# JuanTarrio/rebvo

Hardware: AMD Instinct MI355X
Metric: frames/sec (DoG+extract+track+depth) 752x480 EuRoC (higher is better)
Workload: dtype f32 scale-space / f64 tracker+EKF

## Files before the change

### rebvo_amd/csrc/api.hip

```cpp

#include <math.h>
#include <stdio.h>
#include <stdlib.h>
#include <string.h>

#include <algorithm>
#include <mutex>

#include "ctx.h"
#include "stage_a_dev.h"

namespace edgehip {

static thread_local std::string g_err;

int wait_pinned_ring(edgehip_ctx *c) {
    const int r = c->frames_seen % 8;
    if (c->ring_valid[r]) EH_CHECK(hipEventSynchronize(c->ev_ring[r]));
    return 0;
}

static int wait_idx_row(edgehip_ctx *c, int slot, const int32_t *pi) {
    if (c->slot_src[slot].idx_row != pi) return 0;
    if (c->a_api_valid[slot]) EH_CHECK(hipEventSynchronize(c->ev_a[slot]));
// ... 424 lines not shown
    EH_TRY(dmalloc(c, &c->band_off, B * (nstrips + 1), al->dev, 0));
    {
        char *bs;
        EH_TRY(dmalloc(c, &bs, B * nstrips * c->band_cap * 20, al->dev));
        c->band_stage = bs;
    }
    EH_TRY(dmalloc(c, &c->histo, B * 256, al->dev, 0));
    c->nblk_tvr = (int)((CAP + kTvrBlock - 1) / kTvrBlock);
    EH_TRY(dmalloc(c, &c->P0, B * 3 * CAP, al->dev, 0));
    EH_TRY(dmalloc(c, &c->resid, (size_t)kResidBufs * B * CAP, al->dev, 0));
    EH_TRY(dmalloc(c, &c->resid_carry, (size_t)kResidBufs * B * c->nblk_tvr, al->dev, 0));
    EH_TRY(dmalloc(c, &c->partials, 2 * B * c->nblk_tvr * kNumSums, al->dev, 0));
    EH_TRY(dmalloc(c, &c->block_last, 2 * B * c->nblk_tvr, al->dev, 0));
    EH_TRY(dmalloc(c, &c->bin_cnt, B * 256, al->dev, 0));
    {
        const size_t ntiles = (size_t)((p.w + 63) / 64) * ((p.h + 63) / 64);
        EH_TRY(dmalloc(c, &c->bins, B * ntiles * CAP, al->dev));
    }
    c->field_radius = p.search_range;
    c->field_mode = EH_EXP_ENV("EDGEHIP_FIELD_MODE", 0);
    c->no_grec = getenv("EDGEHIP_NO_GREC") && atoi(getenv("EDGEHIP_NO_GREC")) != 0;
    c->level_mode = getenv("EDGEHIP_LEVEL_MODE") ? atoi(getenv("EDGEHIP_LEVEL_MODE")) : 0;
    c->fwd_mode = EH_EXP_ENV("EDGEHIP_FWD_MODE", 0);
    c->fused_min_batch = fused_min_env;
    c->fused_undist = EH_EXP_ENV("EDGEHIP_FUSED_UNDIST", 0) != 0;
    c->tvr_rw2 = EH_EXP_ENV("EDGEHIP_TVR_RW2", 0);
    c->dual_init = getenv("EDGEHIP_DUAL_INIT") ? atoi(getenv("EDGEHIP_DUAL_INIT")) : 1;
    c->persist_lm_max = EH_EXP_ENV("EDGEHIP_PERSIST_LM", 0);
    EH_TRY(dmalloc(c, &c->sync_cnt, B, al->dev, 0));
    EH_TRY(dmalloc(c, &c->fwd_key, B * CAP, al->dev, 0));
    EH_TRY(dmalloc(c, &c->fwd_win, B * CAP, al->dev, 0xFF));
    EH_TRY(dmalloc(c, &c->rs_tmp, B * 2 * CAP, al->dev, 0));
    c->fuse_match = !(getenv("EDGEHIP_FUSE_MATCH") && atoi(getenv("EDGEHIP_FUSE_MATCH")) == 0);
    if (c->fuse_match) {
        EH_TRY(dmalloc(c, &c->rot_pm, S * B * CAP, al->dev, 0)); EH_TRY(dmalloc(c, &c->rot_mm, S * B * CAP, al->dev, 0));
        EH_TRY(dmalloc(c, &c->rot_rho, S * B * CAP, al->dev, 0)); EH_TRY(dmalloc(c, &c->rot_srho, S * B * CAP, al->dev, 0));
    }
    EH_TRY(dmalloc(c, &c->rot_buf, B * 9, al->dev, 0));
    EH_TRY(dmalloc(c, &c->nav_dev, B, al->dev, 0));
    EH_TRY(dmalloc(c, &c->idx_dev, B, al->dev, 0));
    c->slot_src.assign(S, edgehip_ctx::SlotSrc());
    c->stereo_cnt = nullptr;
    if (p.stereo_available) EH_TRY(dmalloc(c, &c->stereo_cnt, B, al->dev, 0));
    c->nav_log = nullptr;
    c->nav_log_len = 0;

    {
        const size_t al256 = 256;
        auto up = [&](size_t x) { return (x + al256 - 1) / al256 * al256; };
        const bool stereo = p.stereo_available != 0;
        const size_t per = up(CAP * 4) * 8  +
                           up(CAP * 8) * 6  + up(CAP * 8) * 7  + up(CAP * 32) + up(CAP * 16)  +
                           (stereo ? up(CAP * 4) + 2 * up(CAP * 8) : 0);
        char *arena;
        EH_TRY(dmalloc(c, &arena, per * S * B, al->dev, 0));
        c->kl_arena = arena;
        c->kl.resize(S * B);
        for (size_t sb = 0; sb < S * B; sb++) {
            char *q = arena + sb * per;
            KlSoA &k = c->kl[sb];
            auto take = [&](size_t bytes) { char *r = q; q += up(bytes); return r; };
            k.p_inx = (int32_t *)take(CAP * 4);
            k.m_m = (float2 *)take(CAP * 8); k.u_m = (float2 *)take(CAP * 8); k.c_p = (float2 *)take(CAP * 8);
            k.p_m = (float2 *)take(CAP * 8); k.p_m_0 = (float2 *)take(CAP * 8); k.m_m0 = (float2 *)take(CAP * 8);
            k.n_m = (float *)take(CAP * 4);
            k.rho = (double *)take(CAP * 8); k.s_rho = (double *)take(CAP * 8); k.rho_nr = (double *)take(CAP * 8);
// ... 1029 lines not shown
```

### rebvo_amd/csrc/ctx.h

```cpp
#pragma once
#include <hip/hip_runtime.h>
#include <stdint.h>
#include <string.h>
#include <string>
#include <map>
#include <vector>
#include <mutex>
#include <atomic>

#include "edgehip.h"
#include "export_ring.h"

namespace edgehip {

constexpr int kMaxBoxes = 3;
constexpr int kBandRows = 12;
constexpr int kDetWaves = 16;
constexpr int kDivLutMax = 256;
constexpr int kTvrThreads = 256;
constexpr int kTvrPasses = 1;
constexpr int kTvrBlock = kTvrThreads * kTvrPasses;
constexpr int kNumSums = 28;
constexpr int kRefRing = 8;
constexpr int kResidBufs = 3;
// ... 358 lines not shown
    struct SlotSrc { const uint8_t *base = nullptr; std::vector<int32_t> host_idx; bool grey8 = false;
                     const int32_t *idx_row = nullptr; int idx_ring = 0; };
    uint8_t *grey8 = nullptr;
    uint8_t *pinned_grey8 = nullptr;
    std::vector<SlotSrc> slot_src;
    struct SlotCam { float ppx, ppy; double zfm; };
    std::vector<SlotCam> slot_cam;
    int field_radius;
    int field_mode;
    int level_mode;
    int fused_min_batch;
    double pinv_host[3 * 49];
    int32_t *bin_cnt;
    int32_t *bins;
    int nblk_tvr;
    bool fused_undist;
    int tvr_rw2;
    bool tracker_f32 = false;
    int dual_init;
    int persist_lm_max;
    unsigned *sync_cnt;
    unsigned long long *fwd_key;
    int32_t *fwd_win;
    int fwd_mode = 0;
    bool fuse_match = true;
    float2 *rot_pm = nullptr, *rot_mm = nullptr;
    double *rot_rho = nullptr, *rot_srho = nullptr;
    bool rot_pending[4] = {false, false, false, false};
    bool fwd_fill[4] = {false, false, false, false};
    bool fwd_cleared = false;
    bool fwd_keys_posted = false;
    bool fwd_key_in_tvr = false;
    double *rs_tmp;
    double *rot_buf;
    const double *t_src = nullptr;
    edgehip_keyline *aos_dev = nullptr;
    edgehip_keyline *aos_host = nullptr;
    int32_t *aos_req_dev = nullptr, *aos_req_host = nullptr;
    int aos_requests = 0;
    edgehip::ExportRing kl_ring;
    edgehip::ExportRing ros_ring;
    edgehip_nav *nav_dev;
    edgehip_nav *nav_log;
    edgehip_nav_imu *nav_imu_log = nullptr;
    int nav_log_len;
    int32_t *stereo_log = nullptr;
    hipStream_t stream_log = nullptr;
    hipEvent_t ev_log = nullptr;
    hipEvent_t ev_log_ring[8] = {};
    std::mutex log_mu;
    std::atomic<long long> frames_logged{0};
    long long log_first = 0, log_last = -1;
    int32_t *idx_dev;
    int32_t *stereo_cnt;
    uint8_t *pinned_rgb;
    size_t pinned_rgb_bytes;
    edgehip::SeqDev *pinned_seq;
    edgehip::SeqA *pinned_seqa;
    double *pinned_out;
    double *pinned_t;
    int32_t *pinned_idx;
    edgehip_nav *pinned_nav;
    edgehip::Profiler *prof;
    bool imu_enabled = false, imu_pending = false;
    bool imu_pinned_ok = false;
    edgehip_imu_params imu_params;
// ... 84 lines not shown
void drop_frame_graphs(edgehip_ctx *c);
int order_a_after_bc(edgehip_ctx *c);
int order_bc_after_a(edgehip_ctx *c);
int sync_all(edgehip_ctx *c);
int undistort_frame_enqueue(edgehip_ctx *c, int seq, int slot, uint8_t *out_dev);
__device__ inline void frame_begin(SeqDev *sq, double t, double fps) {
    edgehip_seq_state &p = sq->pub;
    double dt = t - p.t_prev;
    if (dt < 0.001) dt = 1 / fps;
    p.dt = dt;
    sq->t_cur = t;
    for (int i = 0; i < 9; i++) {
        const double d = (i == 0 || i == 4 || i == 8) ? 1.0 : 0.0;
        p.P_V[i] = d * 1e50; p.P_W[i] = d * 1e50; p.R[i] = d;
    }
    p.klm_fwd = 0; p.klm_num = 0; p.kf_matchs = 0;
    p.estimation_ok = 1;
    sq->skip_match = 0;
    sq->skip_map = 0;
    p.minimizer_evals = 0;
}

int quantile_enqueue(edgehip_ctx *c, int slot, double smin, double smax, double pct, int nbins, bool frame_begins = false, int retune_slot = -1);
int build_field_enqueue(edgehip_ctx *c, int slot, int radius, float min_mod, bool clear_fwd = false);
int tvr_prepare_enqueue(edgehip_ctx *c, int slot_old, unsigned begin_ops = 0);
int minimizer_enqueue(edgehip_ctx *c, int slot_new, int slot_old, int fc_index);
int minimizer_v_enqueue(edgehip_ctx *c, int slot_new, int slot_old, int fc_index, int iter_max, double match_thresh,
                         uint32_t match_num_thresh, double reweight_distance);
int forward_match_enqueue(edgehip_ctx *c, int slot_old, int slot_new, bool keys_posted = false, bool frame_tail = false);
int forward_rotate_enqueue(edgehip_ctx *c, int slot_old, int slot_new);
int rotate_enqueue(edgehip_ctx *c, int slot, const double *R_host, bool R_in_buf = false);
int rot_materialize_enqueue(edgehip_ctx *c, int slot);
int rec_refresh_enqueue(edgehip_ctx *c, int slot);
int directed_enqueue(edgehip_ctx *c, int slot_new, int slot_old, bool fused = false);
int regekf_enqueue(edgehip_ctx *c, int slot, int do_reg, int do_ekf, bool frame_glue = false);
int rescale_enqueue(edgehip_ctx *c, int slot, bool frame_ends = false);
int pose_enqueue(edgehip_ctx *c, int slot_new, const double *t_host);
int imu_begin_enqueue(edgehip_ctx *c);
int imu_reset_enqueue(edgehip_ctx *c);
int imu_pose_reset_enqueue(edgehip_ctx *c, int seq);
int imu_pre_enqueue(edgehip_ctx *c, int slot_old);
int imu_mid_enqueue(edgehip_ctx *c);
int imu_post_enqueue(edgehip_ctx *c, int slot_new, int have_pair);
void depth_fill_free(edgehip_ctx *c);
int depth_fill_geometry(edgehip_ctx *c, int32_t *gw, int32_t *gh, int32_t *bw, int32_t *bh);
bool depth_fill_grids(edgehip_ctx *c, const double **rho, const double **s_rho);
void depth_surface_free(edgehip_ctx *c);
void net_free(edgehip_ctx *c);
bool net_store(edgehip_ctx *c, const uint8_t **records, const edgehip_net_header **headers, int *kl_size);
void surface_views_free(edgehip_ctx *c);
void ros_free(edgehip_ctx *c);
void kf_track_free(edgehip_ctx *c);
int kf_track_reset_enqueue(edgehip_ctx *c);
int kf_frame_begin_enqueue(edgehip_ctx *c, int slot_old);
int kf_frame_track_enqueue(edgehip_ctx *c, int slot_new);
int kf_frame_end_enqueue(edgehip_ctx *c, int slot_new);

inline int slot_read_done(edgehip_ctx *c, int slot) {
    if (c->stream_a == c->stream) return 0;
    EH_CHECK(hipEventRecord(c->ev_use[slot], c->stream));
    c->use_valid[slot] = true;
    return 0;
}

struct KProfStage {
    double *dev = nullptr, *host = nullptr;
    hipEvent_t ev = nullptr;
    bool busy = false;
// ... 25 lines not shown
```

### rebvo_amd/csrc/stage_c.hip

```cpp

#include <math.h>
#include <string.h>

#include <vector>

#include "ctx.h"
#include "wave_reduce.h"

namespace edgehip {

constexpr double kRhoMax = 20.0, kRhoMin = 1e-3, kRhoInit = 1.0;

__global__ __launch_bounds__(256) void k_fwd_key(const KlSoA *kl_old, const int32_t *__restrict__ kn_old,
                                                 const int32_t *__restrict__ kn_new, unsigned long long *__restrict__ key,
                                                 int cap) {
    const int seq = blockIdx.z, i = blockIdx.x * 256 + threadIdx.x;
    if (i >= kn_old[seq]) return;
    const int f = kl_old[seq].m_id_f[i];
    if (f < 0 || f >= kn_new[seq]) return;
    atomicMax(&key[(size_t)seq * cap + f], ord_bits(kl_old[seq].rho[i]));
}
__device__ inline void so3_exp_c(const double w[3], double R[9]);
__device__ inline void rot_from_state(SeqDev *sq, double *__restrict__ Rbuf_seq);
__device__ inline void glue_after_tracking(SeqDev *sq);
// ... 275 lines not shown
        else { r2[0] = (M[2] + M[6]) / 2; r2[1] = (M[7] + M[5]) / 2; r2[2] = d2; }
        if (r2[0] * r[0] + r2[1] * r[1] + r2[2] * r[2] < 0) { r2[0] = -r2[0]; r2[1] = -r2[1]; r2[2] = -r2[2]; }
        const double nn = sqrt(r2[0] * r2[0] + r2[1] * r2[1] + r2[2] * r2[2]);
        for (int i = 0; i < 3; i++) r[i] = angle * (r2[i] / nn);
    }
}

__device__ inline void rot_from_state(SeqDev *sq, double *__restrict__ Rbuf_seq) {
    double R0[9];
    so3_exp_c(sq->pub.W, R0);
    for (int i = 0; i < 9; i++) Rbuf_seq[i] = R0[i];
    for (int i = 0; i < 3; i++)
        for (int j = 0; j < 3; j++) sq->pub.R[i * 3 + j] = R0[j * 3 + i];
}
__global__ void k_rot_from_state(SeqDev *seqs, double *__restrict__ Rbuf, int nseq) {
    const int seq = blockIdx.x * blockDim.x + threadIdx.x;
    if (seq >= nseq) return;
    rot_from_state(seqs + seq, Rbuf + (size_t)seq * 9);
}

struct DirArgs {
    const KlSoA *kl_new, *kl_old;
    const int32_t *kn_new;
    const int32_t *mask_old;
    SeqDev *seq;
    int w, h;
    size_t n;
    double zfm, min_thr_mod, cang_min_edge, max_radius, loc_unc;
    float ppx, ppy;
    int stereo_mode;
    const int32_t *win;
    RotOut rot;
    int cap;
};

#ifndef EDGEHIP_NT_ROT
#define EDGEHIP_NT_ROT 1
#endif
#ifndef EDGEHIP_NT_EKF
#define EDGEHIP_NT_EKF 1
#endif
#ifndef EDGEHIP_NT_DIRECTED
#define EDGEHIP_NT_DIRECTED 1
#endif
template <bool FUSED, bool FILL>
__device__ __forceinline__ void directed_body(const DirArgs &a) {
    const int seq = blockIdx.z, ik = blockIdx.x * (int)blockDim.x + threadIdx.x;
    SeqDev *sq = a.seq + seq;
    const bool searching = !sq->skip_match;
    if (!FUSED && !searching) return;
    __shared__ double s_v[3], s_rv[9], s_br[9];
    if (threadIdx.x == 0 && searching) {
        const double *BR = sq->pub.R, *V = sq->pub.V, *P = sq->pub.P_V;
        for (int i = 0; i < 9; i++) s_br[i] = BR[i];
        for (int i = 0; i < 3; i++) {
            double d = 0;
            for (int j = 0; j < 3; j++) d += BR[i * 3 + j] * V[j];
            s_v[i] = d;
        }
        double T[9];
        for (int i = 0; i < 3; i++)
            for (int j = 0; j < 3; j++) {
                double d = 0;
                for (int k = 0; k < 3; k++) d += BR[i * 3 + k] * P[k * 3 + j];
                T[i * 3 + j] = d;
            }
        for (int i = 0; i < 3; i++)
            for (int j = 0; j < 3; j++) {
                double d = 0;
                for (int k = 0; k < 3; k++) d += T[i * 3 + k] * BR[j * 3 + k];
                s_rv[i * 3 + j] = d;
            }
    }
    __syncthreads();
    int matched = 0, kfm = 0, fwd = 0;
    if (ik < a.kn_new[seq]) {
        const KlSoA &kn = a.kl_new[seq], &ko = a.kl_old[seq];
        const int32_t *mask = a.mask_old + (size_t)seq * a.n;
        const size_t ro = (size_t)seq * a.cap;
// ... 104 lines not shown
                    const double t = tv[c][dir];
                    jm[c][dir] = -1;
                    if (t0i + c >= t_end) continue;
                    if (dir ? t > dq_max : t < dq_min) continue;
                    const float fx = (float)(t_x * t + (double)pi0x), fy = (float)(t_y * t + (double)pi0y);
                    const int xi = round_half_away_i(fx), yi = round_half_away_i(fy);
                    if (xi >= a.w || yi >= a.h || xi < 0 || yi < 0) continue;
                    jm[c][dir] = mask[__umul24((unsigned)yi, (unsigned)a.w) + (unsigned)xi];
                }
            }
#pragma unroll
            for (int c = 0; c < DM_CH; c++) {
#pragma unroll
                for (int dir = 0; dir < 2; dir++) {
                    const int j = jm[c][dir];
                    if (j < 0 || found >= 0) continue;
                    const double t = tv[c][dir];
                    const float2 omm = FUSED ? ldg(a.rot.m_m, ro + j) : ldg(ko.m_m, j);
                    const double norm_m0 = (double)ldg(ko.n_m, j);
                    const double cang = div_mid((double)(omm.x * kmm.x + omm.y * kmm.y), norm_m0 * norm_m);
                    if (cang < a.cang_min_edge || fabs(norm_m0 / norm_m - 1) > a.min_thr_mod) continue;
                    const double s_rho = FUSED ? ldg(a.rot.s_rho, ro + j) : ldg(ko.s_rho, j), rho = FUSED ? ldg(a.rot.rho, ro + j) : ldg(ko.rho, j);
                    const double v_rho_dr = (a.loc_unc * a.loc_unc + s_rho * s_rho * norm_t * norm_t + sigma2_t * rho * rho);
                    const double dd = t - norm_t * rho;
                    if (dd * dd > v_rho_dr) continue;
                    found = j;
                }
            }
        }
        }
        }
        if (FUSED) {
            const int src = found >= 0 ? found : iw;
            if (src >= 0 || FILL) {
                double rho = kRhoInit, s_rho = kRhoMax, rho_nr = kRhoInit, s_rho_nr = kRhoMax;
                int32_t m_num = -1, m_id_kf = -1;
                float2 pm, mm = make_float2(0.f, 0.f);
                float nm = 0.f;
                if (src < 0) {
                    pm = ldg(kn.p_m, ik);
                } else {
                    const bool turned = found >= 0;
                    rho = turned ? ldg(a.rot.rho, ro + src) : ldg(ko.rho, src);
                    s_rho = turned ? ldg(a.rot.s_rho, ro + src) : ldg(ko.s_rho, src);
                    pm = turned ? ldg(a.rot.p_m, ro + src) : ldg(ko.p_m, src);
                    mm = turned ? ldg(a.rot.m_m, ro + src) : ldg(ko.m_m, src);
                    rho_nr = ldg(ko.rho_nr, src); s_rho_nr = ldg(ko.s_rho_nr, src);
                    m_num = ldg(ko.m_num, src); m_id_kf = ldg(ko.m_id_kf, src);
                    nm = ldg(ko.n_m, src);
                }
#if EDGEHIP_NT_DIRECTED
                stg_stream(kn.rho, ik, rho);
                stg_stream(kn.s_rho, ik, s_rho);
                stg_stream(kn.rho_nr, ik, rho_nr);
                stg_stream(kn.s_rho_nr, ik, s_rho_nr);
                stg_stream(kn.m_num, ik, m_num + 1);
                stg_stream(kn.m_id, ik, src);
                stg_stream(kn.p_m_0, ik, pm);
                stg_stream(kn.m_m0, ik, mm);
                stg_stream(kn.n_m0, ik, (double)nm);
                stg_stream(kn.m_id_kf, ik, m_id_kf);
#else
                stg(kn.rho, ik, rho);
                stg(kn.s_rho, ik, s_rho);
                stg(kn.rho_nr, ik, rho_nr);
                stg(kn.s_rho_nr, ik, s_rho_nr);
                stg(kn.m_num, ik, m_num + 1);
                stg(kn.m_id, ik, src);
                stg(kn.p_m_0, ik, pm);
                stg(kn.m_m0, ik, mm);
                stg(kn.n_m0, ik, (double)nm);
                stg(kn.m_id_kf, ik, m_id_kf);
#endif
                matched = found >= 0;
                kfm = matched && m_id_kf >= 0;
            }
        } else if (found >= 0) {
            const int j = found;
            const double c_rho = a.stereo_mode ? ldg(ko.rho0, j) : ldg(ko.rho, j), c_srho = a.stereo_mode ? ldg(ko.s_rho0, j) : ldg(ko.s_rho, j);
            double c_rho_nr = 0, c_srho_nr = 0;
            if (!a.stereo_mode) { c_rho_nr = ldg(ko.rho_nr, j); c_srho_nr = ldg(ko.s_rho_nr, j); }
            const int32_t c_mnum = ldg(ko.m_num, j), mk = ldg(ko.m_id_kf, j);
            const float2 c_pm = ldg(ko.p_m, j), c_mm = ldg(ko.m_m, j);
            const float c_nm = ldg(ko.n_m, j);
            stg(kn.rho, ik, c_rho);
            stg(kn.s_rho, ik, c_srho);
            if (!a.stereo_mode) {
                stg(kn.rho_nr, ik, c_rho_nr);
                stg(kn.s_rho_nr, ik, c_srho_nr);
            }
            stg(kn.m_id, ik, j);
            stg(kn.m_num, ik, c_mnum + 1);
            stg(kn.p_m_0, ik, c_pm);
            stg(kn.m_m0, ik, c_mm);
            stg(kn.n_m0, ik, (double)c_nm);
            stg(kn.m_id_kf, ik, mk);
            matched = 1;
            kfm = mk >= 0;
        }
    }
    const int c1 = __popcll(__ballot(matched)), c2 = __popcll(__ballot(kfm)), c3 = FUSED ? __popcll(__ballot(fwd)) : 0;
    if ((threadIdx.x & 63) == 0) {
        if (c1) atomicAdd(&sq->pub.klm_num, c1);
        if (c2) atomicAdd(&sq->pub.kf_matchs, c2);
        if (c3) atomicAdd(&sq->pub.klm_fwd, c3);
    }
}
__global__ __launch_bounds__(256) void k_directed(DirArgs a) { directed_body<false, false>(a); }
template <bool FILL>
__global__ __launch_bounds__(256) __attribute__((amdgpu_waves_per_eu(7, 8))) void k_directed_fused(DirArgs a) { directed_body<true, FILL>(a); }


__device__ inline void glue_after_matching(SeqDev *sq);
__global__ __launch_bounds__(256) void k_regularize(const KlSoA *kls, const int32_t *__restrict__ kns, double *__restrict__ rs,
                                                    SeqDev *seqs, int cap, double thresh, int enabled, int match_threshold) {
    const int seq = blockIdx.z, i = blockIdx.x * 256 + threadIdx.x;
    SeqDev *sq = seqs + seq;
    bool skip = sq->skip_map != 0;
    if (match_threshold >= 0 && !sq->skip_match && sq->pub.klm_num < match_threshold) {
        if (i == 0) glue_after_matching(sq);
        skip = true;
    }
    if (skip) return;
    if (i >= kns[seq]) return;
    const KlSoA &K = kls[seq];
    double r = ldg(K.rho, i), s = ldg(K.s_rho, i);
    const int ni = ldg(K.n_id, i), pi = ldg(K.p_id, i);
    if (enabled && ni >= 0 && pi >= 0) {
        const double nrho = ldg(K.rho, ni), prho = ldg(K.rho, pi), nsr = ldg(K.s_rho, ni), psr = ldg(K.s_rho, pi);
        const double d = nrho - prho;
        if (!(d * d > nsr * nsr + psr * psr)) {
            const float2 nm = ldg(K.m_m, ni), pm = ldg(K.m_m, pi);
            double alpha = (double)((nm.x * pm.x + nm.y * pm.y) / (ldg(K.n_m, ni) * ldg(K.n_m, pi)));
            if (!(alpha - thresh < 0)) {
                alpha = (alpha - thresh) / (1 - thresh);
                alpha /= fabs(nrho - prho) / (nsr + psr) + 1;
                const double wr = 1 / (s * s), wrn = alpha / (nsr * nsr), wrp = alpha / (psr * psr);
                const double r2 = (r * wr + nrho * wrn + prho * wrp) / (wr + wrn + wrp);
                const double s2 = (s * wr + nsr * wrn + psr * wrp) / (wr + wrn + wrp);
                r = r2;
                s = s2;
            }
        }
    }
    rs[(size_t)seq * 2 * cap + i] = r;
    rs[(size_t)seq * 2 * cap + cap + i] = s;
}

__global__ __launch_bounds__(256) void k_ekf(const KlSoA *kls, const int32_t *__restrict__ kns, const double *__restrict__ rs,
                                             const SeqDev *seqs, int cap, double zf, double q_abs, double loc_unc, int do_ekf) {
    const int seq = blockIdx.z, i = blockIdx.x * 256 + threadIdx.x;
    const SeqDev *sq = seqs + seq;
    if (sq->skip_map) return;
    if (i >= kns[seq]) return;
    const KlSoA &K = kls[seq];
    double rho = rs[(size_t)seq * 2 * cap + i], s_rho = rs[(size_t)seq * 2 * cap + cap + i];
    if (do_ekf && ldg(K.m_id, i) >= 0) {
        const double v0 = sq->pub.V[0], v1 = sq->pub.V[1], v2 = sq->pub.V[2];
        const double s_rho0 = s_rho;
        const float2 q = ldg(K.p_m, i), q0 = ldg(K.p_m_0, i), mm0 = ldg(K.m_m0, i);
        const double qx = q.x, qy = q.y, q0x = q0.x, q0y = q0.y;
        double v_rho = s_rho * s_rho;
        const double nm0 = ldg(K.n_m0, i);
        const double u_x = (double)mm0.x / nm0, u_y = (double)mm0.y / nm0;
        const double Y = u_x * (qx - q0x) + u_y * (qy - q0y);
        const double H = u_x * (v0 * zf - v2 * q0x) + u_y * (v1 * zf - v2 * q0y);
        const double rho_p = 1 / (1.0 / rho + v2);
        const double rho0 = rho_p;
        double F = 1 / (1 + rho * v2);
        F = F * F;
        const double p_p = F * v_rho * F + q_abs * q_abs;
        const double e = Y - H * rho_p;
        const double S = H * p_p * H + loc_unc * loc_unc;
        const double Kg = p_p * H * (1 / S);
        rho = rho_p + (Kg * e);
        v_rho = (1 - Kg * H) * p_p;
        s_rho = sqrt(v_rho);
        if (rho < kRhoMin) {
            s_rho += kRhoMin - rho;
            rho = kRhoMin;
        } else if (rho > kRhoMax) {
            rho = kRhoMax;
        } else if (isnan(rho) || isnan(s_rho) || isinf(rho) || isinf(s_rho)) {
            rho = kRhoInit;
            s_rho = kRhoMax;
        } else if (s_rho < 0) {
            rho = kRhoInit;
            s_rho = kRhoMax;
        }
#if EDGEHIP_NT_EKF
        stg_stream(K.rho0, i, rho0);
        stg_stream(K.s_rho0, i, s_rho0);
    }
    stg_stream(K.rho, i, rho);
    stg_stream(K.s_rho, i, s_rho);
#else
        stg(K.rho0, i, rho0);
        stg(K.s_rho0, i, s_rho0);
    }
    stg(K.rho, i, rho);
    stg(K.s_rho, i, s_rho);
#endif
}

__device__ __forceinline__ double recip_f64(double x) {
    double y = __builtin_amdgcn_rcp(x);
    y = __builtin_fma(__builtin_fma(-x, y, 1.0), y, y);
    y = __builtin_fma(__builtin_fma(-x, y, 1.0), y, y);
    return y;
}

struct FrameEndArgs {
    edgehip_nav *nav;
    const int32_t *kn_new;
    const double *tresh_new;
    const float *retuned_new;
    edgehip_nav *nav_log;
    int nav_log_len, nseq, have_pair;
};
__device__ inline void frame_end(SeqDev *sq, const int seq, const FrameEndArgs &fe);

template <int NT, int PER, int LJ>
__global__ __launch_bounds__(NT) void k_rescale(const KlSoA *kls, const int32_t *__restrict__ kns, SeqDev *seqs,
                                                double s_rho_min, unsigned match_num_min, int re_escale, FrameEndArgs fe) {
    constexpr int VT = 1024 / NT;
    extern __shared__ double s_tail[];
    const int seq = blockIdx.x, tid = threadIdx.x;
    SeqDev *sq = seqs + seq;
    const int kn = kns[seq];
    bool run = !sq->skip_map;
    if (run && kn <= 0) { if (tid == 0) sq->pub.Kp = 1; run = false; }
    if (run) {
    const KlSoA &K = kls[seq];
    __shared__ double s_a[16], s_b[16];
    __shared__ double s_kp;
    double r2[VT][PER], r02[VT][PER], s2[VT][PER], s02[VT][PER];
// ... 520 lines not shown
                              uy * zf1 * (a.t[1] * den - a.t[2] * (qh1[1] + a.t[1] * srho)) / (den * den);
            double I_rho = (df / a.loc_unc_model) * (df / a.loc_unc_model);
            if (srho != srho || df != df) { srho = 1; I_rho = 1e-10; }
            double ss = 1 / sqrt(I_rho);
            if (srho < 0) { ss = 1e3; srho = 1.0; match = -1; }
            k.stereo_rho[i] = srho;
            k.stereo_s_rho[i] = ss;
        }
        k.stereo_m_id[i] = match;
        matched = match >= 0;
    }
    const int c1 = __popcll(__ballot(matched));
    if ((threadIdx.x & 63) == 0 && c1) atomicAdd(&a.nmatch[seq], c1);
}

__global__ __launch_bounds__(256) void k_fuse_stereo(const KlSoA *kls, const int32_t *__restrict__ kns, SeqDev *seqs) {
    const int seq = blockIdx.z, i = blockIdx.x * 256 + threadIdx.x;
    if (seqs) {
        if (seqs[seq].skip_map) return;
        if (i == 0) seqs[seq].pub.Kp = 1;
    }
    if (i >= kns[seq]) return;
    const KlSoA &k = kls[seq];
    const double r0 = k.rho[i], s0 = k.s_rho[i];
    k.rho0[i] = r0;
    k.s_rho0[i] = s0;
    if (k.stereo_m_id[i] < 0) return;
    const double sr = k.stereo_rho[i], ss = k.stereo_s_rho[i];
    const double s = sqrt(1.0 / (1.0 / (s0 * s0) + 1.0 / (ss * ss)));
    k.s_rho[i] = s;
    k.rho[i] = (r0 / (s0 * s0) + sr / (ss * ss)) * (s * s);
}

int directed_enqueue(edgehip_ctx *c, int slot_new, int slot_old, bool fused) {
    ProfScope ps(c, PROF_C_DIRECTED);
    const DevicePlan &pl = c->plan;
    if (!fused) { if (int e = rot_materialize_enqueue(c, slot_old)) return e; }
    DirArgs a;
    a.kl_new = kldev(c, slot_new); a.kl_old = kldev(c, slot_old);
    a.kn_new = c->kn_slot + (size_t)slot_new * pl.nseq;
    a.mask_old = maskof(c, slot_old);
    a.seq = c->seq; a.w = pl.w; a.h = pl.h; a.n = pl.n; a.zfm = pl.zfm;
    a.min_thr_mod = c->p.match_thresh_module;
    a.cang_min_edge = cos(c->p.match_thresh_angle * M_PI / 180.0);
    a.max_radius = (double)c->p.search_range;
    a.loc_unc = c->p.loc_unc_match;
    a.ppx = pl.ppx; a.ppy = pl.ppy;
    a.stereo_mode = c->p.stereo_available != 0;
    a.win = c->fwd_win; a.cap = pl.cap;
    a.rot = fused ? rot_of(c, slot_old) : RotOut{nullptr, nullptr, nullptr, nullptr};
#ifndef EDGEHIP_DIRECTED_BLOCK
#define EDGEHIP_DIRECTED_BLOCK 128
#endif
    constexpr int kDirBlock = EDGEHIP_DIRECTED_BLOCK;
    const dim3 g((pl.cap + kDirBlock - 1) / kDirBlock, 1, pl.nseq), b(kDirBlock);
    if (fused) {
        if (c->fwd_fill[slot_new]) hipLaunchKernelGGL(k_directed_fused<true>, g, b, 0, c->stream, a);
        else hipLaunchKernelGGL(k_directed_fused<false>, g, b, 0, c->stream, a);
        c->fwd_fill[slot_new] = false;
    } else {
        hipLaunchKernelGGL(k_directed, g, b, 0, c->stream, a);
    }
    EH_LAUNCH_CHECK();
    return 0;
}

int regekf_enqueue(edgehip_ctx *c, int slot, int do_reg, int do_ekf, bool frame_glue) {
    ProfScope ps(c, PROF_C_REGEKF);
    const DevicePlan &pl = c->plan;
    dim3 g((pl.cap + 255) / 256, 1, pl.nseq), b(256);
    const int32_t *kn = c->kn_slot + (size_t)slot * pl.nseq;
    hipLaunchKernelGGL(k_regularize, g, b, 0, c->stream, kldev(c, slot), kn, c->rs_tmp, c->seq, pl.cap,
                       c->p.regularize_thresh, do_reg, frame_glue ? c->p.global_match_threshold : -1);
    hipLaunchKernelGGL(k_ekf, g, b, 0, c->stream, kldev(c, slot), kn, c->rs_tmp, c->seq, pl.cap, pl.zfm, c->p.reshape_q_abs,
                       c->p.loc_unc, do_ekf);
    EH_LAUNCH_CHECK();
    return 0;
}

int rescale_enqueue(edgehip_ctx *c, int slot, bool frame_ends) {
    ProfScope ps(c, PROF_C_RESCALE);
    const DevicePlan &pl = c->plan;
    FrameEndArgs fe = {};
    if (frame_ends) {
        fe.nav = c->nav_dev;
        fe.kn_new = c->kn_slot + (size_t)slot * pl.nseq;
        const int slot_t = c->rig.enabled && c->rig.slot_pair >= 0 ? c->rig.slot_pair : slot;
        fe.tresh_new = c->tresh_slot + (size_t)slot_t * pl.nseq;
        fe.retuned_new = c->retuned_slot + (size_t)slot * pl.nseq;
        fe.nav_log = c->nav_log; fe.nav_log_len = c->nav_log_len; fe.nseq = pl.nseq; fe.have_pair = 1;
    }
    if (!c->lds_optin_rescale) {
        EH_CHECK(hipFuncSetAttribute((const void *)&k_rescale<512, 12, 4>, hipFuncAttributeMaxDynamicSharedMemorySize, 4 * 4 * 1024 * (int)sizeof(double)));
        c->lds_optin_rescale = true;
    }
    hipLaunchKernelGGL((k_rescale<512, 12, 4>), dim3(pl.nseq), dim3(512), 4 * 4 * 1024 * sizeof(double), c->stream, kldev(c, slot),
                       c->kn_slot + (size_t)slot * pl.nseq, c->seq, kRhoMax, 1u, c->p.do_rescaling > 0, fe);
    EH_LAUNCH_CHECK();
    return 0;
}

static int rotate_buf_enqueue(edgehip_ctx *c, int slot) {
    if (int e = rot_materialize_enqueue(c, slot)) return e;
    c->grec_ok[slot] = false;
    c->rec_stale[slot] = true;
    ProfScope ps(c, PROF_C_ROTATE);
// ... 312 lines not shown
        EH_TRY(glue(c, 0, sn, have_pair));
    }
    if (c->imu_enabled) {
        EH_TRY(imu_begin_enqueue(c));
        if (have_pair) {
            EH_TRY(quantile_enqueue(c, so, kRhoMin, kRhoMax, c->p.qcut_quantile, c->p.qcut_nbins, true, retune_in_quantile ? sn : -1));
            EH_TRY(build_field_enqueue(c, sn, c->p.search_range, -1.f, true));
            { ProfScope ps(c, PROF_IMU_FILTERS); EH_TRY(imu_pre_enqueue(c, so)); }
            EH_TRY(rotate_buf_enqueue(c, so));
            {
                ProfScope ps(c, PROF_B_MINIMIZER_V);
                EH_TRY(minimizer_v_enqueue(c, sn, so, c->frames_seen % kRefRing, c->p.tracker_iter_num, c->p.tracker_match_thresh,
                                           c->p.match_num_thresh, c->p.reweight_distance));
            }
            EH_TRY(forward_match_enqueue(c, so, sn, c->fwd_keys_posted));
            c->fwd_keys_posted = false;
            { ProfScope ps(c, PROF_C_EXTROTVEL); EH_TRY(ext_rotvel_enqueue(c, sn)); }
            { ProfScope ps(c, PROF_IMU_FILTERS); EH_TRY(imu_mid_enqueue(c)); }
            EH_TRY(rotate_buf_enqueue(c, so));
            EH_TRY(directed_enqueue(c, sn, so));
            EH_TRY(regekf_enqueue(c, sn, 1, 1, true));
            EH_TRY(rescale_enqueue(c, sn));
        }
        EH_TRY(imu_post_enqueue(c, sn, have_pair));
    } else if (have_pair) {
        if (c->kftrack) EH_TRY(kf_frame_begin_enqueue(c, so));
        EH_TRY(quantile_enqueue(c, so, kRhoMin, kRhoMax, c->p.qcut_quantile, c->p.qcut_nbins, true, retune_in_quantile ? sn : -1));
        EH_TRY(build_field_enqueue(c, sn, c->p.search_range, -1.f, c->fwd_mode != 1));
        c->fwd_key_in_tvr = c->fwd_mode != 1;
        e = minimizer_enqueue(c, sn, so, c->frames_seen % kRefRing);
        c->fwd_key_in_tvr = false;
        if (e) return e;
        const bool one_pass = frame_matches_in_one_pass(c, sp);
#ifdef EDGEHIP_EXPERIMENTS
        if (c->fwd_mode == 2) {
            EH_TRY(forward_rotate_enqueue(c, so, sn));
        } else
#endif
        if (one_pass) {
            EH_TRY(forward_rotate_one_pass_enqueue(c, so, sn));
        } else {
            EH_TRY(forward_match_enqueue(c, so, sn, c->fwd_mode != 1, true));
            EH_TRY(rotate_enqueue(c, so, nullptr, true));
        }
        if (c->fwd_mode == 2) { ProfScope ps(c, PROF_C_POSE); EH_TRY(glue(c, 1, sn, have_pair)); }
        EH_TRY(directed_enqueue(c, sn, so, one_pass));
        if (c->kftrack) EH_TRY(kf_frame_track_enqueue(c, sn));
        EH_TRY(regekf_enqueue(c, sn, 1, 1, true));
        if (sp >= 0) {
            EH_TRY(stereo_enqueue(c, sn, sp, c->rig.t, c->rig.R, c->p.match_thresh_module, c->p.match_thresh_angle, c->rig.max_radius,
                                  c->p.loc_unc_match, c->p.loc_unc, true));
            EH_TRY(fuse_stereo_enqueue(c, sn, true));
        } else {
            EH_TRY(rescale_enqueue(c, sn, true));
            frame_ended = true;
        }
    }
    if (!c->imu_enabled && !frame_ended) {
        ProfScope ps(c, PROF_C_POSE);
        EH_TRY(glue(c, 3, sn, have_pair));
    }
    if (c->kftrack && have_pair && !c->imu_enabled) EH_TRY(kf_frame_end_enqueue(c, sn));
#undef EH_TRY
    for (int s : {sn, so, sp})
        if (s >= 0) { if (int e = slot_read_done(c, s)) return e; }
    return 0;
}

int edgehip_process_frame(edgehip_ctx *c, const double *t) {
    EH_ENTER(c);
    if (!c || !t) return EDGEHIP_ERR_ARG;
    const DevicePlan &pl = c->plan;
    if (c->imu_enabled && !c->imu_pending) { set_error("process_frame: edgehip_set_imu was not called for this frame"); return EDGEHIP_ERR_STATE; }
    const int sn = (c->frame_slot + 1) % c->ring_slots, so = c->frame_slot;
    const int sp = c->rig.enabled ? c->rig.slot_pair : -1;
    const int have_pair = c->frames_seen >= 1;
    double *tp = c->pinned_t + (size_t)(c->frames_seen % 8) * pl.nseq;
    if (int e = wait_pinned_ring(c)) return e;
    memcpy(tp, t, sizeof(double) * pl.nseq);
    const bool profiling = c->prof && c->prof->on;
    const bool graph_path = c->use_graph && !c->overlap && !profiling && c->frames_seen >= 2;
// ... 67 lines not shown
```

Measured before the change: 132,400.

## Fuse regularize and EKF into one kernel via directed-match scratch output

When matching runs in one pass, the fused directed kernel writes rho/s_rho into the rs_tmp scratch buffer instead of the keyline arrays. A single regularize kernel then reads neighbours from scratch, applies regularization and the EKF update, and writes the final values, removing the separate k_ekf launch and one global round trip. The directed kernel gains an extra copy path for unmatched keylines, and the mode is disabled with keyframe tracking.

```diff
diff --git a/rebvo_amd/csrc/api.hip b/rebvo_amd/csrc/api.hip
--- a/rebvo_amd/csrc/api.hip
+++ b/rebvo_amd/csrc/api.hip
@@ -480,6 +480,7 @@
     EH_TRY(dmalloc(c, &c->fwd_win, B * CAP, al->dev, 0xFF));
     EH_TRY(dmalloc(c, &c->rs_tmp, B * 2 * CAP, al->dev, 0));
     c->fuse_match = !(getenv("EDGEHIP_FUSE_MATCH") && atoi(getenv("EDGEHIP_FUSE_MATCH")) == 0);
+    c->regekf_one_pass = !(getenv("EDGEHIP_REGEKF_ONE_PASS") && atoi(getenv("EDGEHIP_REGEKF_ONE_PASS")) == 0);
     if (c->fuse_match) {
         EH_TRY(dmalloc(c, &c->rot_pm, S * B * CAP, al->dev, 0)); EH_TRY(dmalloc(c, &c->rot_mm, S * B * CAP, al->dev, 0));
         EH_TRY(dmalloc(c, &c->rot_rho, S * B * CAP, al->dev, 0)); EH_TRY(dmalloc(c, &c->rot_srho, S * B * CAP, al->dev, 0));
diff --git a/rebvo_amd/csrc/ctx.h b/rebvo_amd/csrc/ctx.h
--- a/rebvo_amd/csrc/ctx.h
+++ b/rebvo_amd/csrc/ctx.h
@@ -414,6 +414,7 @@
     bool fwd_keys_posted = false;
     bool fwd_key_in_tvr = false;
     double *rs_tmp;
+    bool regekf_one_pass = true;
     double *rot_buf;
     const double *t_src = nullptr;
     edgehip_keyline *aos_dev = nullptr;
@@ -564,8 +565,8 @@
 int rotate_enqueue(edgehip_ctx *c, int slot, const double *R_host, bool R_in_buf = false);
 int rot_materialize_enqueue(edgehip_ctx *c, int slot);
 int rec_refresh_enqueue(edgehip_ctx *c, int slot);
-int directed_enqueue(edgehip_ctx *c, int slot_new, int slot_old, bool fused = false);
-int regekf_enqueue(edgehip_ctx *c, int slot, int do_reg, int do_ekf, bool frame_glue = false);
+int directed_enqueue(edgehip_ctx *c, int slot_new, int slot_old, bool fused = false, bool pair_to_scratch = false);
+int regekf_enqueue(edgehip_ctx *c, int slot, int do_reg, int do_ekf, bool frame_glue = false, bool from_scratch = false);
 int rescale_enqueue(edgehip_ctx *c, int slot, bool frame_ends = false);
 int pose_enqueue(edgehip_ctx *c, int slot_new, const double *t_host);
 int imu_begin_enqueue(edgehip_ctx *c);
diff --git a/rebvo_amd/csrc/stage_c.hip b/rebvo_amd/csrc/stage_c.hip
--- a/rebvo_amd/csrc/stage_c.hip
+++ b/rebvo_amd/csrc/stage_c.hip
@@ -331,6 +331,7 @@
     const int32_t *win;
     RotOut rot;
     int cap;
+    double *rs;
 };
 
 #ifndef EDGEHIP_NT_ROT
@@ -342,8 +343,33 @@
 #ifndef EDGEHIP_NT_DIRECTED
 #define EDGEHIP_NT_DIRECTED 1
 #endif
-template <bool FUSED, bool FILL>
+#ifndef EDGEHIP_NT_RS_SCRATCH
+#define EDGEHIP_NT_RS_SCRATCH 0
+#endif
+template <bool RS>
+__device__ __forceinline__ void store_matched_pair(const DirArgs &a, const KlSoA &kn, int seq, int ik, double rho, double s_rho) {
+    if (RS) {
+        double *r = a.rs + (size_t)seq * 2 * a.cap;
+#if EDGEHIP_NT_RS_SCRATCH
+        stg_stream(r, ik, rho);
+        stg_stream(r, (size_t)a.cap + ik, s_rho);
+#else
+        stg(r, ik, rho);
+        stg(r, (size_t)a.cap + ik, s_rho);
+#endif
+    } else {
+#if EDGEHIP_NT_DIRECTED
+        stg_stream(kn.rho, ik, rho);
+        stg_stream(kn.s_rho, ik, s_rho);
+#else
+        stg(kn.rho, ik, rho);
+        stg(kn.s_rho, ik, s_rho);
+#endif
+    }
+}
+template <bool FUSED, bool FILL, bool RS = false>
 __device__ __forceinline__ void directed_body(const DirArgs &a) {
+    static_assert(FUSED || !RS, "the scratch destination belongs to matching in one pass");
     const int seq = blockIdx.z, ik = blockIdx.x * (int)blockDim.x + threadIdx.x;
     SeqDev *sq = a.seq + seq;
     const bool searching = !sq->skip_match;
@@ -514,7 +540,10 @@
         }
         if (FUSED) {
             const int src = found >= 0 ? found : iw;
-            if (src >= 0 || FILL) {
+            if (RS && !FILL && src < 0) {
+                const double rho = ldg(kn.rho, ik), s_rho = ldg(kn.s_rho, ik);
+                store_matched_pair<true>(a, kn, seq, ik, rho, s_rho);
+            } else if (src >= 0 || FILL) {
                 double rho = kRhoInit, s_rho = kRhoMax, rho_nr = kRhoInit, s_rho_nr = kRhoMax;
                 int32_t m_num = -1, m_id_kf = -1;
                 float2 pm, mm = make_float2(0.f, 0.f);
@@ -531,9 +560,8 @@
                     m_num = ldg(ko.m_num, src); m_id_kf = ldg(ko.m_id_kf, src);
                     nm = ldg(ko.n_m, src);
                 }
+                store_matched_pair<RS>(a, kn, seq, ik, rho, s_rho);
 #if EDGEHIP_NT_DIRECTED
-                stg_stream(kn.rho, ik, rho);
-                stg_stream(kn.s_rho, ik, s_rho);
                 stg_stream(kn.rho_nr, ik, rho_nr);
                 stg_stream(kn.s_rho_nr, ik, s_rho_nr);
                 stg_stream(kn.m_num, ik, m_num + 1);
@@ -543,8 +571,6 @@
                 stg_stream(kn.n_m0, ik, (double)nm);
                 stg_stream(kn.m_id_kf, ik, m_id_kf);
 #else
-                stg(kn.rho, ik, rho);
-                stg(kn.s_rho, ik, s_rho);
                 stg(kn.rho_nr, ik, rho_nr);
                 stg(kn.s_rho_nr, ik, s_rho_nr);
                 stg(kn.m_num, ik, m_num + 1);
@@ -589,27 +615,16 @@
     }
 }
 __global__ __launch_bounds__(256) void k_directed(DirArgs a) { directed_body<false, false>(a); }
-template <bool FILL>
-__global__ __launch_bounds__(256) __attribute__((amdgpu_waves_per_eu(7, 8))) void k_directed_fused(DirArgs a) { directed_body<true, FILL>(a); }
+template <bool FILL, bool RS>
+__global__ __launch_bounds__(256) __attribute__((amdgpu_waves_per_eu(7, 8))) void k_directed_fused(DirArgs a) { directed_body<true, FILL, RS>(a); }
 
 
 __device__ inline void glue_after_matching(SeqDev *sq);
-__global__ __launch_bounds__(256) void k_regularize(const KlSoA *kls, const int32_t *__restrict__ kns, double *__restrict__ rs,
-                                                    SeqDev *seqs, int cap, double thresh, int enabled, int match_threshold) {
-    const int seq = blockIdx.z, i = blockIdx.x * 256 + threadIdx.x;
-    SeqDev *sq = seqs + seq;
-    bool skip = sq->skip_map != 0;
-    if (match_threshold >= 0 && !sq->skip_match && sq->pub.klm_num < match_threshold) {
-        if (i == 0) glue_after_matching(sq);
-        skip = true;
-    }
-    if (skip) return;
-    if (i >= kns[seq]) return;
-    const KlSoA &K = kls[seq];
-    double r = ldg(K.rho, i), s = ldg(K.s_rho, i);
+__device__ __forceinline__ void regularize_1(const KlSoA &K, const double *__restrict__ R, const double *__restrict__ S, int i,
+                                             double thresh, double &r, double &s) {
     const int ni = ldg(K.n_id, i), pi = ldg(K.p_id, i);
-    if (enabled && ni >= 0 && pi >= 0) {
-        const double nrho = ldg(K.rho, ni), prho = ldg(K.rho, pi), nsr = ldg(K.s_rho, ni), psr = ldg(K.s_rho, pi);
+    if (ni >= 0 && pi >= 0) {
+        const double nrho = ldg(R, ni), prho = ldg(R, pi), nsr = ldg(S, ni), psr = ldg(S, pi);
         const double d = nrho - prho;
         if (!(d * d > nsr * nsr + psr * psr)) {
             const float2 nm = ldg(K.m_m, ni), pm = ldg(K.m_m, pi);
@@ -625,18 +640,9 @@
             }
         }
     }
-    rs[(size_t)seq * 2 * cap + i] = r;
-    rs[(size_t)seq * 2 * cap + cap + i] = s;
-}
-
-__global__ __launch_bounds__(256) void k_ekf(const KlSoA *kls, const int32_t *__restrict__ kns, const double *__restrict__ rs,
-                                             const SeqDev *seqs, int cap, double zf, double q_abs, double loc_unc, int do_ekf) {
-    const int seq = blockIdx.z, i = blockIdx.x * 256 + threadIdx.x;
-    const SeqDev *sq = seqs + seq;
-    if (sq->skip_map) return;
-    if (i >= kns[seq]) return;
-    const KlSoA &K = kls[seq];
-    double rho = rs[(size_t)seq * 2 * cap + i], s_rho = rs[(size_t)seq * 2 * cap + cap + i];
+}
+__device__ __forceinline__ void ekf_store(const KlSoA &K, const SeqDev *sq, int i, double rho, double s_rho, double zf, double q_abs,
+                                          double loc_unc, int do_ekf) {
     if (do_ekf && ldg(K.m_id, i) >= 0) {
         const double v0 = sq->pub.V[0], v1 = sq->pub.V[1], v2 = sq->pub.V[2];
         const double s_rho0 = s_rho;
@@ -684,6 +690,52 @@
     stg(K.s_rho, i, s_rho);
 #endif
 }
+template <bool ONE_PASS>
+__global__ __launch_bounds__(256) void k_regularize(const KlSoA *kls, const int32_t *__restrict__ kns, double *__restrict__ rs,
+                                                    SeqDev *seqs, int cap, double thresh, int enabled, int match_threshold,
+                                                    double zf, double q_abs, double loc_unc, int do_ekf) {
+    const int seq = blockIdx.z, i = blockIdx.x * 256 + threadIdx.x;
+    SeqDev *sq = seqs + seq;
+    bool skip = sq->skip_map != 0;
+    if (match_threshold >= 0 && !sq->skip_match && sq->pub.klm_num < match_threshold) {
+        if (i == 0) glue_after_matching(sq);
+        skip = true;
+    }
+    if (!ONE_PASS && skip) return;
+    if (i >= kns[seq]) return;
+    const KlSoA &K = kls[seq];
+    double *R = rs + (size_t)seq * 2 * cap, *S = R + cap;
+    if (ONE_PASS) {
+        double r = ldg(R, i), s = ldg(S, i);
+        if (skip) {
+#if EDGEHIP_NT_EKF
+            stg_stream(K.rho, i, r);
+            stg_stream(K.s_rho, i, s);
+#else
+            stg(K.rho, i, r);
+            stg(K.s_rho, i, s);
+#endif
+            return;
+        }
+        if (enabled) regularize_1(K, R, S, i, thresh, r, s);
+        ekf_store(K, sq, i, r, s, zf, q_abs, loc_unc, do_ekf);
+    } else {
+        double r = ldg(K.rho, i), s = ldg(K.s_rho, i);
+        if (enabled) regularize_1(K, K.rho, K.s_rho, i, thresh, r, s);
+        R[i] = r;
+        S[i] = s;
+    }
+}
+
+__global__ __launch_bounds__(256) void k_ekf(const KlSoA *kls, const int32_t *__restrict__ kns, const double *__restrict__ rs,
+                                             const SeqDev *seqs, int cap, double zf, double q_abs, double loc_unc, int do_ekf) {
+    const int seq = blockIdx.z, i = blockIdx.x * 256 + threadIdx.x;
+    const SeqDev *sq = seqs + seq;
+    if (sq->skip_map) return;
+    if (i >= kns[seq]) return;
+    const double rho = rs[(size_t)seq * 2 * cap + i], s_rho = rs[(size_t)seq * 2 * cap + cap + i];
+    ekf_store(kls[seq], sq, i, rho, s_rho, zf, q_abs, loc_unc, do_ekf);
+}
 
 __device__ __forceinline__ double recip_f64(double x) {
     double y = __builtin_amdgcn_rcp(x);
@@ -1270,7 +1322,7 @@
     k.rho[i] = (r0 / (s0 * s0) + sr / (ss * ss)) * (s * s);
 }
 
-int directed_enqueue(edgehip_ctx *c, int slot_new, int slot_old, bool fused) {
+int directed_enqueue(edgehip_ctx *c, int slot_new, int slot_old, bool fused, bool pair_to_scratch) {
     ProfScope ps(c, PROF_C_DIRECTED);
     const DevicePlan &pl = c->plan;
     if (!fused) { if (int e = rot_materialize_enqueue(c, slot_old)) return e; }
@@ -1287,14 +1339,22 @@
     a.stereo_mode = c->p.stereo_available != 0;
     a.win = c->fwd_win; a.cap = pl.cap;
     a.rot = fused ? rot_of(c, slot_old) : RotOut{nullptr, nullptr, nullptr, nullptr};
+    if (pair_to_scratch && !fused) { set_error("directed_matching: the scratch destination needs matching in one pass"); return EDGEHIP_ERR_STATE; }
+    a.rs = pair_to_scratch ? c->rs_tmp : nullptr;
 #ifndef EDGEHIP_DIRECTED_BLOCK
 #define EDGEHIP_DIRECTED_BLOCK 128
 #endif
     constexpr int kDirBlock = EDGEHIP_DIRECTED_BLOCK;
     const dim3 g((pl.cap + kDirBlock - 1) / kDirBlock, 1, pl.nseq), b(kDirBlock);
     if (fused) {
-        if (c->fwd_fill[slot_new]) hipLaunchKernelGGL(k_directed_fused<true>, g, b, 0, c->stream, a);
-        else hipLaunchKernelGGL(k_directed_fused<false>, g, b, 0, c->stream, a);
+        const bool fill = c->fwd_fill[slot_new];
+        if (pair_to_scratch) {
+            if (fill) hipLaunchKernelGGL((k_directed_fused<true, true>), g, b, 0, c->stream, a);
+            else hipLaunchKernelGGL((k_directed_fused<false, true>), g, b, 0, c->stream, a);
+        } else {
+            if (fill) hipLaunchKernelGGL((k_directed_fused<true, false>), g, b, 0, c->stream, a);
+            else hipLaunchKernelGGL((k_directed_fused<false, false>), g, b, 0, c->stream, a);
+        }
         c->fwd_fill[slot_new] = false;
     } else {
         hipLaunchKernelGGL(k_directed, g, b, 0, c->stream, a);
@@ -1303,13 +1363,20 @@
     return 0;
 }
 
-int regekf_enqueue(edgehip_ctx *c, int slot, int do_reg, int do_ekf, bool frame_glue) {
+int regekf_enqueue(edgehip_ctx *c, int slot, int do_reg, int do_ekf, bool frame_glue, bool from_scratch) {
     ProfScope ps(c, PROF_C_REGEKF);
     const DevicePlan &pl = c->plan;
     dim3 g((pl.cap + 255) / 256, 1, pl.nseq), b(256);
     const int32_t *kn = c->kn_slot + (size_t)slot * pl.nseq;
-    hipLaunchKernelGGL(k_regularize, g, b, 0, c->stream, kldev(c, slot), kn, c->rs_tmp, c->seq, pl.cap,
-                       c->p.regularize_thresh, do_reg, frame_glue ? c->p.global_match_threshold : -1);
+    const int match_threshold = frame_glue ? c->p.global_match_threshold : -1;
+    if (from_scratch) {
+        hipLaunchKernelGGL(k_regularize<true>, g, b, 0, c->stream, kldev(c, slot), kn, c->rs_tmp, c->seq, pl.cap, c->p.regularize_thresh,
+                           do_reg, match_threshold, pl.zfm, c->p.reshape_q_abs, c->p.loc_unc, do_ekf);
+        EH_LAUNCH_CHECK();
+        return 0;
+    }
+    hipLaunchKernelGGL(k_regularize<false>, g, b, 0, c->stream, kldev(c, slot), kn, c->rs_tmp, c->seq, pl.cap, c->p.regularize_thresh,
+                       do_reg, match_threshold, pl.zfm, c->p.reshape_q_abs, c->p.loc_unc, do_ekf);
     hipLaunchKernelGGL(k_ekf, g, b, 0, c->stream, kldev(c, slot), kn, c->rs_tmp, c->seq, pl.cap, pl.zfm, c->p.reshape_q_abs,
                        c->p.loc_unc, do_ekf);
     EH_LAUNCH_CHECK();
@@ -1688,6 +1755,7 @@
         c->fwd_key_in_tvr = false;
         if (e) return e;
         const bool one_pass = frame_matches_in_one_pass(c, sp);
+        const bool reg_one_pass = one_pass && c->regekf_one_pass && !c->kftrack;
 #ifdef EDGEHIP_EXPERIMENTS
         if (c->fwd_mode == 2) {
             EH_TRY(forward_rotate_enqueue(c, so, sn));
@@ -1700,9 +1768,9 @@
             EH_TRY(rotate_enqueue(c, so, nullptr, true));
         }
         if (c->fwd_mode == 2) { ProfScope ps(c, PROF_C_POSE); EH_TRY(glue(c, 1, sn, have_pair)); }
-        EH_TRY(directed_enqueue(c, sn, so, one_pass));
+        EH_TRY(directed_enqueue(c, sn, so, one_pass, reg_one_pass));
         if (c->kftrack) EH_TRY(kf_frame_track_enqueue(c, sn));
-        EH_TRY(regekf_enqueue(c, sn, 1, 1, true));
+        EH_TRY(regekf_enqueue(c, sn, 1, 1, true, reg_one_pass));
         if (sp >= 0) {
             EH_TRY(stereo_enqueue(c, sn, sp, c->rig.t, c->rig.R, c->p.match_thresh_module, c->p.match_thresh_angle, c->rig.max_radius,
                                   c->p.loc_unc_match, c->p.loc_unc, true));
```

Result: no change. 132,400 (-0.0%).
